# e-c-k-e-r/tortoise-tts

Hardware: AMD Instinct MI355X
Metric: audio-sec/wall-sec (RTF^-1), 16 AR candidates x 80 DDIM steps (higher is better)
Workload: dtype bf16; 1 GPU; configs[1]: 1 utterance/GPU, 64 text tokens, 16 AR candidates x 250 mel tokens (KV-cached decode), latent pass on 16 candidates, 80 DDIM steps with cond-free guidance at T=1088 (11.6 s audio); candidates=16, ddim_steps=80, mel_frames=1088, parallelism=single GPU, small_models=False, vocoder_in_step=False

## Files before the change

### tortoise_tts_amd/csrc/gemm.hip

```cpp
#include <stdlib.h>

#include <type_traits>

#include <hip/hip_ext.h>

#include "gemm_epilogue.h"

namespace ttk {

template <typename T, int BM, int NWM, int NWN, int ROLE>
__device__ __forceinline__ void conv3_image_tile(const GemmParams& p, const int m0, const int n0, const int wave) {
	typedef GRole<ROLE> R;
	static_assert(R::on && R::CONV && R::RES && sizeof(T) == 2, "the k = 3 residual role on 16-bit operands");
	constexpr int ES = 2, BN = 64, KSTEPS = 2, NW = NWM * NWN;
	constexpr int WM = BM / NWM, WN = BN / NWN, MI = WM / 16, NI = WN / 16;
	static_assert(MI == 4 && NI == 2, "64 x 32 wave blocks");
	constexpr int IMG_ROWS = BM + 8, IMG = IMG_ROWS * 128, NPA = IMG_ROWS / 8;
	constexpr int A_PC = (NPA + NW - 1) / NW, B_PC = 8 / NW;
	constexpr int NB = 4, BT = BN * 128, OFF_B = 2 * IMG, OFF_DUMP = OFF_B + NB * BT;
	constexpr int KC = GR_K / 64, NM = KSTEPS * MI * NI, NR = KSTEPS * (MI + NI), RPG = TTK_PIPE_RPG, D0 = TTK_PIPE_D0;
	static_assert(KC % 2 == 0 && (NR + RPG - 1) / RPG <= NM && D0 + B_PC + A_PC <= NM, "reads and DMA pieces must fit the MFMA gaps");
	constexpr unsigned TAPB = (unsigned)(R::N * GR_K * ES);
	constexpr int RESN = MI * 4 * NI;
	constexpr unsigned OOR = 0x80000000u;
	extern __shared__ __attribute__((aligned(16))) char smem[];
	const int lane = threadIdx.x & 63, g = lane >> 4, l15 = lane & 15;
#ifdef TTK_STAMPS
	unsigned long long* const stamps_ = p.stamps;
#endif
	const int wm = wave / NWN, wn = wave % NWN;
	const unsigned smem_base = __builtin_amdgcn_readfirstlane(lds_addr(smem));
	const int Tb = p.rows_per_batch;
	float bias_pre[NI];
#pragma unroll
	for (int j = 0; j < NI; ++j) bias_pre[j] = p.bias[n0 + wn * WN + 16 * j + l15];

	unsigned fa[3][KSTEPS], fb[KSTEPS];
#pragma unroll
	for (int ks = 0; ks < KSTEPS; ++ks) {
#pragma unroll
		for (int sg = 0; sg < 3; ++sg) {
			const int r = wm * WM + l15 + sg;
			fa[sg][ks] = smem_base + r * 128 + (((4 * ks + g) ^ (r & 7)) << 4);
		}
		const int rowb = wn * WN + l15;
		fb[ks] = smem_base + OFF_B + rowb * 128 + (((4 * ks + g) ^ (rowb & 7)) << 4);
	}
	const int prow = lane >> 3, pslot = lane & 7;
	unsigned va[A_PC], vb[B_PC];
#pragma unroll
	for (int i = 0; i < A_PC; ++i) {
		const int q = wave + NW * i, r = 8 * q + prow, gr = m0 - 1 + r;
		const bool ok = q < NPA && r < BM + 2 && gr >= 0 && gr < p.M;
		va[i] = ok ? (unsigned)(gr * (GR_K * ES) + ((pslot ^ (r & 7)) << 4)) : OOR;
	}
#pragma unroll
	for (int i = 0; i < B_PC; ++i) {
		const int row = 8 * (wave + NW * i) + prow;
		vb[i] = (unsigned)((n0 + row) * (GR_K * ES) + ((pslot ^ (row & 7)) << 4));
	}
	const __amdgpu_buffer_rsrc_t srdB = __builtin_amdgcn_make_buffer_rsrc((void*)p.W, 0, 0x7fffffff, 0x00020000);
	const __amdgpu_buffer_rsrc_t srdA = __builtin_amdgcn_make_buffer_rsrc((void*)p.seg[0].A, 0, (unsigned)p.M * (unsigned)(GR_K * ES), 0x00020000);
	int mlo = 0, mhi = 0;
#pragma unroll
	for (int i = 0; i < MI; ++i) {
		const int x = m0 + wm * WM + 16 * i + l15;
		const int t = x - div_recip(x, Tb, p.inv_rpb) * Tb;
		mlo |= (t == 0 ? 1 : 0) << i;
		mhi |= (t == Tb - 1 ? 1 : 0) << i;
	}
	const bool any_lo = __builtin_amdgcn_ballot_w64(mlo != 0) != 0, any_hi = __builtin_amdgcn_ballot_w64(mhi != 0) != 0;

	struct PFrags { u32x4 a[KSTEPS][MI], b[KSTEPS][NI]; };
	f32x4 acc[MI][NI];
#pragma unroll
	for (int i = 0; i < MI; ++i)
#pragma unroll
		for (int j = 0; j < NI; ++j) acc[i][j] = f32x4{0.f, 0.f, 0.f, 0.f};

	auto issue_image = [&](auto i_, auto slot_, unsigned kc) {
		constexpr int i = decltype(i_)::value, slot = decltype(slot_)::value;
		const int q = wave + NW * i;
		pipe_glds16(va[i], srdA, kc * 128u, q < NPA ? smem_base + slot * IMG + q * 1024 : smem_base + OFF_DUMP);
	};
	auto issue_w = [&](auto i_, unsigned soff, unsigned slot_off) {
		constexpr int i = decltype(i_)::value;
		pipe_glds16(vb[i], srdB, soff, smem_base + OFF_B + slot_off + (wave + NW * i) * 1024);
	};
	auto read_one = [&](auto r_, auto slot_, auto s_, PFrags& fr, const unsigned (&rb)[KSTEPS]) {
		constexpr int r = decltype(r_)::value, ks = r / (MI + NI), q = r % (MI + NI), SLOT = decltype(slot_)::value, S = decltype(s_)::value;
		if constexpr (q < MI) pipe_read16<q * 2048 + SLOT * IMG>(fr.a[ks][q], fa[S][ks]);
		else pipe_read16<(q - MI) * 2048>(fr.b[ks][q - MI], rb[ks]);
	};
	auto clear_edges = [&](auto s_, PFrags& fr) {
		constexpr int S = decltype(s_)::value;
		if constexpr (S == 0 || S == 2) {
			if (S == 0 ? any_lo : any_hi) {
				const int m = S == 0 ? mlo : mhi;
#pragma unroll
				for (int i = 0; i < MI; ++i) {
					const bool z = (m >> i) & 1;
// ... 15 lines not shown
		unsigned rb[KSTEPS];
#pragma unroll
		for (int ks = 0; ks < KSTEPS; ++ks) rb[ks] = fb[ks] + rd_slot;
		const unsigned soffW = (unsigned)S_CUR * TAPB + kc_w * 128u;
		if constexpr (RD || PER > 0) { wait_vmcnt<W>(); pipe_barrier(); }
		static_for<0, NM>([&](auto m_) {
			constexpr int m = decltype(m_)::value, ks = m / (MI * NI), i = (m % (MI * NI)) / NI, j = m % NI;
			pipe_mfma<T>(acc[i][j], cur.a[ks][i], cur.b[ks][j]);
			if constexpr (RD) static_for<0, RPG>([&](auto q_) {
				constexpr int r = m * RPG + decltype(q_)::value;
				if constexpr (r < NR) read_one(std::integral_constant<int, r>{}, slot_rd_, s_rd_, nxt, rb);
			});
			if constexpr (PER > 0 && m >= D0 && m - D0 < PER) {
				constexpr int d = m - D0;
				if constexpr (ISW && d < B_PC) issue_w(std::integral_constant<int, d>{}, soffW, wr_slot);
				else issue_image(std::integral_constant<int, d - (ISW ? B_PC : 0)>{}, slot_w_, kc_i);
			}
		});
		if constexpr (RD) { pipe_lgkm0(); clear_edges(s_rd_, nxt); }
		tb = (tb + 1) & 3;
	};
	typedef std::integral_constant<int, 0> I0; typedef std::integral_constant<int, 1> I1; typedef std::integral_constant<int, 2> I2;
	typedef std::true_type Y; typedef std::false_type N;

	PipeScope scope = pipe_begin();
	static_for<0, A_PC>([&](auto i_) { issue_image(i_, I0{}, 0u); });
	static_for<0, 3>([&](auto t_) { static_for<0, B_PC>([&](auto i_) { issue_w(i_, (unsigned)decltype(t_)::value * TAPB, (unsigned)decltype(t_)::value * BT); }); });
	static_for<0, A_PC>([&](auto i_) { issue_image(i_, I1{}, 1u); });
	TTK_WSTAMP(stamps_, blockIdx.x, 1);
	wait_vmcnt<2 * B_PC + A_PC>();
	pipe_barrier();
	TTK_WSTAMP(stamps_, blockIdx.x, 2);
	PFrags f0, f1;
	{
		unsigned rb0[KSTEPS];
#pragma unroll
		for (int ks = 0; ks < KSTEPS; ++ks) rb0[ks] = fb[ks];
		static_for<0, NR>([&](auto r_) { read_one(r_, I0{}, I0{}, f0, rb0); });
	}
	pipe_lgkm0();
	clear_edges(I0{}, f0);
	scope.clk = kclock_start();
	typedef std::integral_constant<int, B_PC + A_PC> W01; typedef std::integral_constant<int, B_PC> W2;
	const int row0 = m0 + wm * WM, col0 = n0 + wn * WN;
	float res_pre[MI][4][NI];
	for (int kc = 0; kc < KC - 2; kc += 2) {
		trip(W01{}, Y{}, I0{}, I1{}, Y{}, I0{}, N{}, I0{}, f0, f1, (unsigned)kc + 1, 0u);
		trip(W01{}, Y{}, I0{}, I2{}, Y{}, I1{}, N{}, I0{}, f1, f0, (unsigned)kc + 1, 0u);
		trip(W2{}, Y{}, I1{}, I0{}, Y{}, I2{}, Y{}, I0{}, f0, f1, (unsigned)kc + 1, (unsigned)kc + 2);
		trip(W01{}, Y{}, I1{}, I1{}, Y{}, I0{}, N{}, I1{}, f1, f0, (unsigned)kc + 2, 0u);
		trip(W01{}, Y{}, I1{}, I2{}, Y{}, I1{}, N{}, I1{}, f0, f1, (unsigned)kc + 2, 0u);
		trip(W2{}, Y{}, I0{}, I0{}, Y{}, I2{}, Y{}, I1{}, f1, f0, (unsigned)kc + 2, (unsigned)kc + 3);
	}
	{
		constexpr unsigned kc = KC - 2;
		trip(W01{}, Y{}, I0{}, I1{}, Y{}, I0{}, N{}, I0{}, f0, f1, kc + 1, 0u);
		trip(W01{}, Y{}, I0{}, I2{}, Y{}, I1{}, N{}, I0{}, f1, f0, kc + 1, 0u);
		trip(W2{}, Y{}, I1{}, I0{}, Y{}, I2{}, N{}, I0{}, f0, f1, kc + 1, 0u);
		if (m0 + BM <= p.M) load_residual_role<ROLE, MI, NI, false>(p, res_pre, row0, col0, lane);
		else load_residual_role<ROLE, MI, NI, true>(p, res_pre, row0, col0, lane);
		asm volatile("" ::: "memory");
		TTK_FENCE();
		trip(std::integral_constant<int, B_PC + RESN>{}, Y{}, I1{}, I1{}, N{}, I0{}, N{}, I1{}, f1, f0, 0u, 0u);
		trip(std::integral_constant<int, RESN>{}, Y{}, I1{}, I2{}, N{}, I1{}, N{}, I1{}, f0, f1, 0u, 0u);
		trip(I0{}, N{}, I0{}, I0{}, N{}, I2{}, N{}, I0{}, f1, f0, 0u, 0u);
	}
	pipe_end(scope, TTK_GEMM_STAMPS(p), lane);
	TTK_WSTAMPD(stamps_, blockIdx.x, 3, acc[0][0][0]);
	if (m0 + BM <= p.M) epilogue_role<T, ROLE, false, MI, NI, true>(p, acc, res_pre, bias_pre, row0, col0, lane);
	else epilogue_role<T, ROLE, true, MI, NI, true>(p, acc, res_pre, bias_pre, row0, col0, lane);
	TTK_WSTAMP(stamps_, blockIdx.x, 4);
#if defined(TTK_STAMPS) && TTK_STAMPS == 2
	asm volatile("s_waitcnt vmcnt(0)" ::: "memory");
	TTK_WSTAMP(stamps_, blockIdx.x, 5);
#endif
}

template <typename T, int BM, int BN, int NWM, int NWN, int NSTAGE, int ROLE, bool LONGK = false>
__device__ __forceinline__ void gemm_tile(const GemmParams& p, const int m0, const int n0, const int wave) {
	typedef GRole<ROLE> R;
	static_assert(!R::on || (sizeof(T) <= 2 && R::N % BN == 0), "roles are 16-bit or fp8, N a multiple of the tile width");
	constexpr int LDS_AVAIL = NSTAGE * ((BM == 64 && NWM == 1 ? 128 : BM) + BN) * 128;
	if constexpr (TTK_CONV_IMAGE && R::on && R::CONV && sizeof(T) == 2 && BN == 64 && NWN == 2 && BM / NWM == 64 && LDS_AVAIL >= 2 * (BM + 8) * 128 + 4 * 8192 + 1024) {
		conv3_image_tile<T, BM, NWM, NWN, ROLE>(p, m0, n0, wave);
		return;
	}
	constexpr int ES = sizeof(T);
	constexpr bool F8 = ES == 1;
	constexpr int BKE = 128 / ES;
	constexpr int KSTEPS = F8 ? 2 : BKE / 32;
	constexpr int FCH = F8 ? 1 : 8 * ES / 16;
	constexpr int EPC = 16 / ES;
	constexpr int NW = NWM * NWN;
	constexpr int WM = BM / NWM, WN = BN / NWN, MI = WM / 16, NI = WN / 16;
	constexpr int A_PC = BM / 8 / NW, B_PC = BN / 8 / NW;
	static_assert(A_PC >= 1 && B_PC >= 1 && A_PC * 8 * NW == BM && B_PC * 8 * NW == BN, "tile does not split into 1-KiB pieces per wave");
	constexpr int PER_TILE = A_PC + B_PC;
	constexpr int STAGE = (BM + BN) * 128;
	typedef typename Frag<T>::type FragT;
	extern __shared__ __attribute__((aligned(16))) char smem[];
	const int tid = threadIdx.x, lane = tid & 63;
#ifdef TTK_STAMPS
	unsigned long long* const stamps_ = p.stamps;
#endif
	const int wm = wave / NWN, wn = wave % NWN;
	const int KT = R::on ? GR_K / BKE : p.K / BKE;
	const int NTILES = R::on ? R::NSEG * KT : p.nseg * KT;

	const int prow = lane >> 3, pslot = lane & 7;
	int a_gm[A_PC], a_t[A_PC];
#pragma unroll
	for (int i = 0; i < A_PC; ++i) {
		a_gm[i] = m0 + 8 * (wave + NW * i) + prow;
		if constexpr (R::on) a_t[i] = R::CONV ? a_gm[i] - div_recip(a_gm[i], p.rows_per_batch, p.inv_rpb) * p.rows_per_batch : 0;
		else a_t[i] = p.rows_per_batch > 0 ? a_gm[i] % p.rows_per_batch : 0;
	}
	const unsigned smem_base = __builtin_amdgcn_readfirstlane(lds_addr(smem));
	constexpr unsigned OOR = 0x80000000u;
	unsigned va[A_PC], vb[B_PC];
#pragma unroll
	for (int i = 0; i < B_PC; ++i) {
		const int row = 8 * (wave + NW * i) + prow;
		const int c = pslot ^ (row & 7);
		if constexpr (R::on) vb[i] = (unsigned)((n0 + row) * (GR_K * ES) + c * 16);
		else vb[i] = (unsigned)(((int64_t)(n0 + row) * p.ldw + c * EPC) * ES);
	}
	const __amdgpu_buffer_rsrc_t srdB = __builtin_amdgcn_make_buffer_rsrc((void*)p.W, 0, 0x7fffffff, 0x00020000);
	__amdgpu_buffer_rsrc_t srdA = srdB;
	unsigned b_seg_off = 0;
	int seg_i = 0, kk_i = 0;
	const bool seg_in = R::on ? R::CONV : (p.seg_inner != 0);
	const int NSEG = R::on ? R::NSEG : p.nseg;
	unsigned va3[R::CONV ? 3 : 1][A_PC];
	if constexpr (R::on && R::CONV) {
#pragma unroll
		for (int sg = 0; sg < 3; ++sg)
#pragma unroll
			for (int i = 0; i < A_PC; ++i) {
				const int row = 8 * (wave + NW * i) + prow;
				const int c = pslot ^ (row & 7);
				const int t = a_t[i] + sg - 1;
				const bool ok = a_gm[i] < p.M && t >= 0 && t < p.rows_per_batch;
				va3[sg][i] = ok ? (unsigned)((a_gm[i] + sg - 1) * (GR_K * ES) + c * 16) : OOR;
			}
		srdA = __builtin_amdgcn_make_buffer_rsrc((void*)p.seg[0].A, 0, (unsigned)p.M * (unsigned)(GR_K * ES), 0x00020000);
	}
	auto set_segment = [&](int sg) {
		if constexpr (R::on && R::CONV) {
			b_seg_off = (unsigned)sg * (unsigned)(R::N * GR_K * ES);
#pragma unroll
			for (int i = 0; i < A_PC; ++i) va[i] = sg == 0 ? va3[0][i] : (sg == 1 ? va3[1][i] : va3[2][i]);
			return;
		}
		if constexpr (R::on) {
			srdA = __builtin_amdgcn_make_buffer_rsrc((void*)p.seg[0].A, 0, (unsigned)p.M * (unsigned)(GR_K * ES), 0x00020000);
			b_seg_off = 0;
#pragma unroll
			for (int i = 0; i < A_PC; ++i) {
				const int row = 8 * (wave + NW * i) + prow;
				const int c = pslot ^ (row & 7);
				va[i] = a_gm[i] < p.M ? (unsigned)(a_gm[i] * (GR_K * ES) + c * 16) : OOR;
			}
			return;
		}
		sg = __builtin_amdgcn_readfirstlane(sg);
		const int64_t lda = p.seg[sg].lda;
		const int shift = p.seg[sg].shift;
// ... 351 lines not shown
			asm volatile("s_waitcnt lgkmcnt(0)" ::: "memory");
	#endif
	#if !(defined(TTK_DIAG_SKIP) && (TTK_DIAG_SKIP & 64))
			__builtin_amdgcn_s_barrier();
	#endif
			asm volatile("" ::: "memory");
	#ifdef TTK_DIAG_SKIP
			if ((TTK_DIAG_SKIP & 4) && kt > 0) { if (kt + NSTAGE < NTILES) issue(kt % NSTAGE); mfma_tile(cur); return; }
			if ((TTK_DIAG_SKIP & 8) && kt > 0) { if (kt + NSTAGE < NTILES) issue(kt % NSTAGE); read_frags(nxt, (kt + 1) % NSTAGE); return; }
	#endif
			if (kt + NSTAGE < NTILES) issue(kt % NSTAGE);
			read_frags(nxt, (kt + 1) % NSTAGE);
			mfma_tile(cur);
		};

	#pragma unroll
		for (int st = 0; st < NSTAGE; ++st)
			if (st < NTILES) issue(st);
		TTK_WSTAMP(stamps_, blockIdx.x, 1);
		wait_tiles(min(NSTAGE, NTILES) - 1);
		__builtin_amdgcn_s_barrier();
		asm volatile("" ::: "memory");
		TTK_WSTAMP(stamps_, blockIdx.x, 2);
		Frags f0, f1;
		read_frags(f0, 0);
		if constexpr (PRE_RES) {
			constexpr int NT = R::NSEG * (GR_K / BKE);
			static_assert(!PRE_RES || (NT % 2 == 0 && NT >= 8), "the peeled tail assumes an even tile count");
			auto tail_step = [&](auto wtag, int stage_next, const Frags& cur, Frags& nxt) {
				wait_vmcnt<decltype(wtag)::value>();
	#if !(defined(TTK_DIAG_SKIP) && (TTK_DIAG_SKIP & 32))
				asm volatile("s_waitcnt lgkmcnt(0)" ::: "memory");
	#endif
				__builtin_amdgcn_s_barrier();
				asm volatile("" ::: "memory");
				read_frags(nxt, stage_next);
				mfma_tile(cur);
			};
			int kt = 0;
			for (; kt < NT - 4; kt += 2) {
				step(kt, f0, f1);
				step(kt + 1, f1, f0);
			}
			step(NT - 4, f0, f1);
			if (m0 + BM <= p.M) load_residual_role<ROLE, MI, NI, false>(p, res_pre, row0, col0, lane);
			else load_residual_role<ROLE, MI, NI, true>(p, res_pre, row0, col0, lane);
			asm volatile("" ::: "memory");
			tail_step(std::integral_constant<int, PER_TILE + RESN>{}, (NT - 2) % NSTAGE, f1, f0);
			tail_step(std::integral_constant<int, RESN>{}, (NT - 1) % NSTAGE, f0, f1);
			mfma_tile(f1);
		} else {
			int kt = 0;
			for (; kt + 2 < NTILES; kt += 2) {
				step(kt, f0, f1);
				step(kt + 1, f1, f0);
			}
			if (kt + 2 == NTILES) { step(kt, f0, f1); mfma_tile(f1); }
			else mfma_tile(f0);
		}
	}
	TTK_WSTAMPD(stamps_, blockIdx.x, 3, acc[0][0][0]);

	if constexpr (R::on) {
		if (m0 + BM <= p.M) epilogue_role<T, ROLE, false, MI, NI, PRE_RES>(p, acc, res_pre, bias_pre, row0, col0, lane);
		else epilogue_role<T, ROLE, true, MI, NI, PRE_RES>(p, acc, res_pre, bias_pre, row0, col0, lane);
		TTK_WSTAMP(stamps_, blockIdx.x, 4);
#if defined(TTK_STAMPS) && TTK_STAMPS == 2
		asm volatile("s_waitcnt vmcnt(0)" ::: "memory");
		TTK_WSTAMP(stamps_, blockIdx.x, 5);
#endif
		return;
	}
	const bool full = (m0 + BM <= p.M) && (n0 + BN <= p.N);
	if (p.transpose_out) { if (full) epilogue<T, 2, false, MI, NI>(p, acc, row0, col0, lane); else epilogue<T, 2, true, MI, NI>(p, acc, row0, col0, lane); }
	else if (p.out_f32) { if (full) epilogue<T, 1, false, MI, NI>(p, acc, row0, col0, lane); else epilogue<T, 1, true, MI, NI>(p, acc, row0, col0, lane); }
	else { if (full) epilogue<T, 0, false, MI, NI>(p, acc, row0, col0, lane); else epilogue<T, 0, true, MI, NI>(p, acc, row0, col0, lane); }
	TTK_WSTAMP(stamps_, blockIdx.x, 4);
#if defined(TTK_STAMPS) && TTK_STAMPS == 2
	asm volatile("s_waitcnt vmcnt(0)" ::: "memory");
	TTK_WSTAMP(stamps_, blockIdx.x, 5);
#endif
}

template <typename B> __device__ __forceinline__ int xcd_tile_id(B block, int nwg) {
	const int xcd = block & 7, q = nwg >> 3, r = nwg & 7;
	return (xcd < r ? xcd * (q + 1) : r * (q + 1) + (xcd - r) * q) + (block >> 3);
}

template <typename T, int BM, int BN, int NWM, int NWN, int NSTAGE, int ROLE = GR_NONE, bool LONGK = false>
__global__ __launch_bounds__(64 * NWM * NWN, 2) void k_gemm(GemmParams p) {
	typedef GRole<ROLE> R;

	if constexpr (R::on) {
		if constexpr (R::CONV) TTK_PIN_ARGS(TTK_S(p.M), TTK_S(p.W), TTK_S(p.seg[0].A), TTK_S(p.tiles_m), TTK_S(p.inv_tiles_m), TTK_S(p.rows_per_batch), TTK_S(p.inv_rpb));
		else TTK_PIN_ARGS(TTK_S(p.M), TTK_S(p.W), TTK_S(p.seg[0].A), TTK_S(p.tiles_m), TTK_S(p.inv_tiles_m));
	} else {
		TTK_PIN_ARGS(TTK_S(p.M), TTK_S(p.N), TTK_S(p.K), TTK_S(p.nseg), TTK_S(p.W), TTK_S(p.ldw), TTK_S(p.rows_per_batch), TTK_S(p.m_major),
					 TTK_S(p.seg[0].A), TTK_S(p.seg[0].lda), TTK_S(p.seg[0].shift), TTK_S(p.seg[0].w_off));
	}
	const int wave = __builtin_amdgcn_readfirstlane((int)threadIdx.x >> 6);
#ifdef TTK_STAMPS
	unsigned long long* const stamps_ = p.stamps;
#endif
	TTK_WSTAMP(stamps_, blockIdx.x, 0);
	const int tiles_m = R::on ? p.tiles_m : (p.M + BM - 1) / BM;
	const int tile_id = xcd_tile_id(blockIdx.x, R::on ? tiles_m * (R::N / BN) : (int)gridDim.x);
	int m0, n0;
	if constexpr (R::on) {
		const int tn = div_recip(tile_id, tiles_m, p.inv_tiles_m);
		m0 = (tile_id - tn * tiles_m) * BM; n0 = tn * BN;
	} else {
		const int tiles_n = (p.N + BN - 1) / BN;
		m0 = p.m_major ? (tile_id / tiles_n) * BM : (tile_id % tiles_m) * BM;
		n0 = p.m_major ? (tile_id % tiles_n) * BN : (tile_id / tiles_m) * BN;
	}
	gemm_tile<T, BM, BN, NWM, NWN, NSTAGE, ROLE, LONGK>(p, m0, n0, wave);
}

template <typename T, int ROLE>
__global__ __launch_bounds__(256, 2) void k_gemm_mixed(GemmParams p) {
	typedef GRole<ROLE> R;
	static_assert(R::on && R::N == 1024, "mixed grids serve the 1024-wide roles");
	if constexpr (R::CONV) TTK_PIN_ARGS(TTK_S(p.M), TTK_S(p.W), TTK_S(p.seg[0].A), TTK_S(p.mix_full), TTK_S(p.mix_fm), TTK_S(p.inv_tiles_m),
										TTK_S(p.rows_per_batch), TTK_S(p.inv_rpb));
	else TTK_PIN_ARGS(TTK_S(p.M), TTK_S(p.W), TTK_S(p.seg[0].A), TTK_S(p.mix_full), TTK_S(p.mix_fm), TTK_S(p.inv_tiles_m));
	const int wave = __builtin_amdgcn_readfirstlane((int)threadIdx.x >> 6);
#ifdef TTK_STAMPS
	unsigned long long* const stamps_ = p.stamps;
#endif
	TTK_WSTAMP(stamps_, blockIdx.x, 0);
	const int b = blockIdx.x;
	if (b < p.mix_full) {
		const int tile_id = xcd_tile_id(b, p.mix_full);
		const int tn = div_recip(tile_id, p.mix_fm, p.inv_tiles_m);
		gemm_tile<T, 128, 64, 2, 2, TTK_ROLE_STAGES, ROLE>(p, (tile_id - tn * p.mix_fm) * 128, tn * 64, wave);
	} else {
		if (wave >= 2) return;
		const int j = b - p.mix_full;
		gemm_tile<T, 64, 64, 1, 2, TTK_ROLE_STAGES, ROLE>(p, p.mix_fm * 128 + (j >> 4) * 64, (2 * (j & 7) + ((j >> 3) & 1)) * 64, wave);
	}
}

static void opt_in_lds_once(bool& done, const void* kernel, int lds) {
	if (done) return;
	if (lds > 64 * 1024) (void)hipFuncSetAttribute(kernel, hipFuncAttributeMaxDynamicSharedMemorySize, lds);
	done = true;
}
static void fill_derived(GemmParams& p, int tiles_m) {
	p.tiles_m = tiles_m;
	p.inv_tiles_m = 1.0f / (float)tiles_m;
	p.inv_rpb = p.rows_per_batch > 0 ? 1.0f / (float)p.rows_per_batch : 0.f;
	p.inv_gn_T = p.gn_T > 0 ? 1.0f / (float)p.gn_T : 0.f;
}

template <typename T, int BM, int BN, int NWM, int NWN, int NSTAGE, int ROLE = GR_NONE, bool LONGK = false>
static void launch_tile(const GemmParams& p_in, hipStream_t s, hipEvent_t ea, hipEvent_t eb) {
	constexpr int LDS = NSTAGE * (BM + BN) * 128;
	if constexpr (!LONGK && ROLE == GR_NONE && sizeof(T) == 2 && BM == 256 && BN == 128 && NSTAGE == 3) {
		if (TTK_GEMM_PIPE_H && (p_in.K / 64) * p_in.nseg > NSTAGE) return launch_tile<T, BM, BN, NWM, NWN, NSTAGE, ROLE, true>(p_in, s, ea, eb);
	}
	static bool attr_set = false;
	opt_in_lds_once(attr_set, (const void*)k_gemm<T, BM, BN, NWM, NWN, NSTAGE, ROLE, LONGK>, LDS);
	GemmParams p = p_in;
	fill_derived(p, (p.M + BM - 1) / BM);
	const int grid = p.tiles_m * ((p.N + BN - 1) / BN);
	hipExtLaunchKernelGGL((k_gemm<T, BM, BN, NWM, NWN, NSTAGE, ROLE, LONGK>), dim3(grid), dim3(64 * NWM * NWN), (unsigned)LDS, s, ea, eb, 0, p);
}

static int g_mixed_mode = -1;
static bool mixed_grid_applies(const GemmParams& p) {
	if (g_mixed_mode < 0) { const char* e = getenv("TTK_GEMM_MIXED"); g_mixed_mode = e ? atoi(e) : 1; }
	if (!g_mixed_mode || p.N != 1024 || p.M % 64 != 0) return false;
	const int tiles_m = (p.M + 127) / 128;
	return tiles_m * 16 > 256 && tiles_m * 16 <= 320;
}
template <typename T, int ROLE>
static void launch_mixed(const GemmParams& p_in, hipStream_t s, hipEvent_t ea, hipEvent_t eb) {
	constexpr int LDS = TTK_ROLE_STAGES * (128 + 64) * 128;
	static_assert(LDS > 64 * 1024, "the mixed grid's ring needs the LDS opt-in");
	static bool attr_set = false;
	opt_in_lds_once(attr_set, (const void*)k_gemm_mixed<T, ROLE>, LDS);
	GemmParams p = p_in;
	p.mix_fm = 16; p.mix_full = 256;
	fill_derived(p, p.mix_fm);
	const int blocks64 = (p.M - 128 * p.mix_fm) / 64;
	hipExtLaunchKernelGGL((k_gemm_mixed<T, ROLE>), dim3(p.mix_full + blocks64 * 16), dim3(256), (unsigned)LDS, s, ea, eb, 0, p);
}

int g_gemm_roles = -1;
void gemm_roles_refresh() {
	g_mixed_mode = -1;
	const char* e = getenv("TTK_GEMM_ROLE");
	g_gemm_roles = e ? (atoi(e) == 1 ? 0x1E : atoi(e)) : 0x1E;
}
static int gemm_role_of_unmasked(const GemmParams& p, int es);
static int gemm_role_of(const GemmParams& p, int es) {
	const int r = gemm_role_of_unmasked(p, es);
	return (g_gemm_roles >> r) & 1 ? r : GR_NONE;
}
static int gemm_role_of_unmasked(const GemmParams& p, int es) {
	if (g_gemm_roles < 0) gemm_roles_refresh();
	if ((es != 2 && es != 1) || p.K != GR_K || p.ldw != GR_K || !p.bias || p.act != ACT_NONE || (es == 2) != (p.out_scale == 0.f)) return GR_NONE;
	if (p.transpose_out || p.m_major) return GR_NONE;
	if (p.M < 1 || p.M > (1 << 19) || p.seg[0].lda != GR_K || p.seg[0].w_off != 0) return GR_NONE;
	if (p.nseg == 1 && p.seg[0].shift == 0) {
		if (p.N == 3072 && !p.out_f32 && p.ldc == 3072 && !p.residual && !p.gn_part) return GR_QKV;
		if (p.N == 1024 && p.out_f32 && p.ldc == 1024 && p.gn_part && p.gn_T > 0) return !p.residual ? GR_IN1x1 : (p.ldr == 1024 ? GR_PROJ_RES : GR_NONE);
		return GR_NONE;
	}
	if (p.nseg == 3 && p.N == 1024 && p.out_f32 && p.ldc == 1024 && p.residual && p.ldr == 1024 && p.gn_part && p.gn_T > 0 && p.rows_per_batch > 0) {
		for (int j = 0; j < 3; ++j)
			if (p.seg[j].A != p.seg[0].A || p.seg[j].lda != GR_K || p.seg[j].shift != j - 1 || p.seg[j].w_off != (int64_t)j * 1024 * GR_K) return GR_NONE;
		return GR_CONV3_RES;
	}
	return GR_NONE;
}
static bool is_stat_role(int role) { return role == GR_IN1x1 || role == GR_CONV3_RES || role == GR_PROJ_RES; }
template <typename F> static void with_stat_role(int role, F&& f) {
	if (role == GR_IN1x1) f(std::integral_constant<int, GR_IN1x1>{});
	else if (role == GR_CONV3_RES) f(std::integral_constant<int, GR_CONV3_RES>{});
	else if (role == GR_PROJ_RES) f(std::integral_constant<int, GR_PROJ_RES>{});
}
template <typename T, int BM, int BN, int NWM, int NWN, int NSTAGE>
static void launch_tile_role(int role, const GemmParams& p, hipStream_t s, hipEvent_t ea, hipEvent_t eb) {
	if constexpr (sizeof(T) <= 2) {
		if constexpr (BM == 128 && BN == 64) {
			if (is_stat_role(role) && mixed_grid_applies(p)) return with_stat_role(role, [&](auto r) { launch_mixed<T, decltype(r)::value>(p, s, ea, eb); });
		}
		constexpr int NS = (BM == 128 && BN == 64 && sizeof(T) == 2) ? TTK_ROLE_STAGES : NSTAGE;
		if constexpr (BN <= 128) {
			if (is_stat_role(role)) return with_stat_role(role, [&](auto r) { launch_tile<T, BM, BN, NWM, NWN, NS, decltype(r)::value>(p, s, ea, eb); });
		}
		if (role == GR_QKV) return launch_tile<T, BM, BN, NWM, NWN, NS, GR_QKV>(p, s, ea, eb);
	}
	launch_tile<T, BM, BN, NWM, NWN, NSTAGE>(p, s, ea, eb);
}

int g_force_tile = -1;
static void read_force_tile() { if (g_force_tile < 0) { const char* e = getenv("TTK_GEMM_TILE"); g_force_tile = e ? atoi(e) + 100 : 99; } }
static int pick_tile(int M, int N) {
	const int t128 = ((M + 127) / 128) * ((N + 127) / 128);
	const int t12864 = ((M + 127) / 128) * ((N + 63) / 64);
	return t128 >= 256 ? 0 : (t12864 >= 128 ? 1 : 2);
}
bool gemm_fuses_gn_stats(int M, int N, int C, int T) {
	read_force_tile();
	if (g_force_tile >= 100 && g_force_tile - 100 == 2) return false;
	return C == 1024 && N == C && T % 64 == 0 && M % 64 == 0 && pick_tile(M, N) != 2;
}

template <typename T>
static void launch_gemm_t(const GemmParams& p, hipStream_t s, hipEvent_t ea, hipEvent_t eb) {
	read_force_tile();
	int tile;
	if (g_force_tile >= 100) tile = g_force_tile - 100;
	else {
		tile = pick_tile(p.M, p.N);
	}
	static const int wide = [] { const char* e = getenv("TTK_GEMM_TILE_WIDE"); return e ? atoi(e) : -2; }();
	if (g_force_tile < 100 && tile == 0) {
		const int t128 = ((p.M + 127) / 128) * ((p.N + 127) / 128), t256 = ((p.M + 255) / 256) * ((p.N + 127) / 128);
		if (wide >= 0) { if (p.N >= 3072) tile = wide; }
		else if (wide == -2 && sizeof(T) <= 2 && t128 > 256) {
			const int r128 = (t128 + 255) / 256, r256 = (t256 + 255) / 256;
			if (15 * r256 <= 9 * r128) tile = 8;
		}
	}
	const int role = gemm_role_of(p, (int)sizeof(T));
	if (tile == 0) launch_tile_role<T, 128, 128, 2, 4, 3>(role, p, s, ea, eb);
	else if (tile == 1) launch_tile_role<T, 128, 64, 2, 2, 3>(role, p, s, ea, eb);
	else if (tile == 3) launch_tile<T, 128, 128, 2, 4, 4>(p, s, ea, eb);
	else if (tile == 4) launch_tile<T, 128, 64, 2, 2, 5>(p, s, ea, eb);
	else if (tile == 5) launch_tile<T, 128, 64, 4, 2, 3>(p, s, ea, eb);
	else if (tile == 6) launch_tile<T, 128, 64, 2, 4, 3>(p, s, ea, eb);
	else if (tile == 7) launch_tile<T, 256, 64, 4, 2, 3>(p, s, ea, eb);
	else if (tile == 8) launch_tile_role<T, 256, 128, 4, 2, 3>(role, p, s, ea, eb);
	else if (tile == 9) launch_tile<T, 128, 128, 2, 4, 2>(p, s, ea, eb);
	else launch_tile<T, 64, 64, 2, 2, 3>(p, s, ea, eb);
}

void launch_gemm(int dt, const GemmParams& p_in, hipStream_t s) {
	static const int order = [] { const char* e = getenv("TTK_GEMM_ORDER"); return e ? atoi(e) : 0; }();
	GemmParams p = p_in;
	if (order == 1) p.m_major = p.nseg == 1 && (int64_t)p.N < p.M;
	else if (order == 2) p.m_major = (int64_t)p.N * p.nseg < p.M;
	else if (order == 3) p.m_major = 1;
	p.seg_inner = p.nseg == 3 && p.seg[0].shift == -1 && p.seg[1].shift == 0 && p.seg[2].shift == 1 && p.seg[1].A == p.seg[0].A && p.seg[2].A == p.seg[0].A &&
				  p.seg[1].lda == p.seg[0].lda && p.seg[2].lda == p.seg[0].lda;
	hipEvent_t ea = nullptr, eb = nullptr;
	if (g_prof_on) prof_pair(PROF_GEMM, 2.0 * p.M * p.N * (double)p.K * p.nseg, &ea, &eb);
	if (dt == DT_FP8) launch_gemm_t<f8>(p, s, ea, eb);
	else if (dt == DT_BF16) launch_gemm_t<bf16>(p, s, ea, eb);
	else if (dt == DT_F16) launch_gemm_t<f16>(p, s, ea, eb);
	else launch_gemm_t<float>(p, s, ea, eb);
}

}
```

### tortoise_tts_amd/csrc/gemm_prims.h

```cpp
#pragma once

#include <type_traits>

#include "ttk_common.h"
#include "ttk_kernels.h"

#ifndef TTK_GEMM_PIPE
#define TTK_GEMM_PIPE 1
#endif
#ifndef TTK_GEMM_PIPE_H
#define TTK_GEMM_PIPE_H 1
#endif
#ifndef TTK_CONV_IMAGE
#define TTK_CONV_IMAGE 1
#endif
#ifndef TTK_ROLE_STAGES
#define TTK_ROLE_STAGES 3
#endif
#ifndef TTK_FP8_SCALED_MFMA
#define TTK_FP8_SCALED_MFMA 1
#endif
#ifndef TTK_PIPE_RPG
#define TTK_PIPE_RPG 2
#endif
#ifndef TTK_PIPE_PREB
#define TTK_PIPE_PREB 0
#endif
#ifndef TTK_PIPE_DPG
#define TTK_PIPE_DPG 1
#endif
#ifndef TTK_PIPE_DLATE
#define TTK_PIPE_DLATE 0
#endif
#ifndef TTK_PIPE_D0
#define TTK_PIPE_D0 6
#endif

#ifdef TTK_STAMPS
#define TTK_GEMM_STAMPS(p) ((p).stamps)
#else
#define TTK_GEMM_STAMPS(p) ((unsigned long long*)nullptr)
#endif

namespace ttk {

__device__ __forceinline__ void glds16(unsigned voff, __amdgpu_buffer_rsrc_t srd, unsigned soff, unsigned lds_dst ) {
	unsigned keep;
	asm volatile("s_mov_b32 %0, m0\n\ts_mov_b32 m0, %1\n\ts_nop 0\n\tbuffer_load_dwordx4 %2, %3, %4 offen lds\n\ts_mov_b32 m0, %0"
				 : "=&s"(keep) : "s"(lds_dst), "v"(voff), "s"(srd), "s"(soff) : "memory");
}
__device__ __forceinline__ unsigned lds_addr(const void* p) {
	return (unsigned)(uintptr_t)(const __attribute__((address_space(3))) char*)p;
}
template <int N> __device__ __forceinline__ void wait_vmcnt() { asm volatile("s_waitcnt vmcnt(%0)" ::"n"(N) : "memory"); }
template <int I, int N, typename F> __device__ __forceinline__ void static_for(F&& f) {
	if constexpr (I < N) { f(std::integral_constant<int, I>{}); static_for<I + 1, N>(f); }
}

typedef __attribute__((ext_vector_type(4))) unsigned u32x4;
#define TTK_FENCE() __builtin_amdgcn_sched_barrier(0)
template <int OFF> __device__ __forceinline__ void pipe_read16(u32x4& d, unsigned addr) {
	static_assert(OFF >= 0 && OFF < 65536, "ds_read offset field");
	asm volatile("ds_read_b128 %0, %1 offset:%2" : "=v"(d) : "v"(addr), "n"(OFF));
	TTK_FENCE();
}
template <typename T> __device__ __forceinline__ void pipe_mfma(f32x4& c, const u32x4& a, const u32x4& b) {
	union U { u32x4 q; typename Frag<T>::type v; __device__ U() {} } ua, ub;
	ua.q = a; ub.q = b;
	c = mma16<T>(ua.v, ub.v, c);
	TTK_FENCE();
}
__device__ __forceinline__ void pipe_lgkm0() { asm volatile("s_waitcnt lgkmcnt(0)" ::: "memory"); TTK_FENCE(); }
__device__ __forceinline__ void pipe_barrier() { TTK_FENCE(); __builtin_amdgcn_s_barrier(); asm volatile("" ::: "memory"); TTK_FENCE(); }
__device__ __forceinline__ void pipe_glds16(unsigned voff, __amdgpu_buffer_rsrc_t srd, unsigned soff, unsigned lds_dst ) {
	asm volatile("s_mov_b32 m0, %0\n\ts_nop 0\n\tbuffer_load_dwordx4 %1, %2, %3 offen lds" :: "s"(lds_dst), "v"(voff), "s"(srd), "s"(soff) : "memory");
	TTK_FENCE();
}
#ifdef TTK_CLOCK_STAMPS
struct KClock { unsigned long long clk0, rt0; };
__device__ __forceinline__ KClock kclock_start() { return KClock{__builtin_amdgcn_s_memtime(), __builtin_amdgcn_s_memrealtime()}; }
__device__ __forceinline__ void kclock_stop(const KClock& c, unsigned long long* stamps, int lane) {
	if (stamps && lane == 0) {
		unsigned long long* st_ = stamps + ((size_t)blockIdx.x * 16 + (threadIdx.x >> 6)) * 8;
		st_[6] = ((__builtin_amdgcn_s_memtime() - c.clk0) << 32) | ((__builtin_amdgcn_s_memrealtime() - c.rt0) & 0xffffffffull);
	}
}
#else
struct KClock {};
__device__ __forceinline__ KClock kclock_start() { return KClock{}; }
__device__ __forceinline__ void kclock_stop(const KClock&, unsigned long long*, int) {}
#endif
__device__ __forceinline__ unsigned pipe_m0_save() { unsigned k; asm volatile("s_mov_b32 %0, m0" : "=s"(k)); TTK_FENCE(); return k; }
__device__ __forceinline__ void pipe_m0_restore(unsigned k) { asm volatile("s_mov_b32 m0, %0" :: "s"(k)); TTK_FENCE(); }
struct PipeScope { unsigned m0_keep; KClock clk; };
__device__ __forceinline__ PipeScope pipe_begin() {
	PipeScope s;
	asm volatile("s_mov_b32 %0, m0" : "=s"(s.m0_keep));
	TTK_FENCE();
	return s;
}
// ... 8 lines not shown
```

### tortoise_tts_amd/csrc/ttk_kernels.h

```cpp
#pragma once
#include <hip/hip_runtime.h>
#include <stdint.h>

namespace ttk {

enum DType { DT_F32 = 0, DT_BF16 = 1, DT_FP8W = 2, DT_FP8 = 3, DT_F16 = 4 };
inline int elem_kind(int dt) { return dt == DT_F32 ? 1 : (dt == DT_F16 ? 2 : 0); }
inline size_t dtype_size(int dt) { return dt == DT_F32 ? 4 : 2; }
inline int kernel_dtype(int dt) { return (dt == DT_FP8W || dt == DT_FP8) ? DT_BF16 : dt; }

enum ProfKind { PROF_GEMM = 0, PROF_SKINNY = 1, PROF_ATTN_FWD = 2, PROF_ATTN_DECODE = 3, PROF_GN_STATS = 4, PROF_GN_APPLY = 5,
				PROF_LAYERNORM = 6, PROF_KINDS = 7 };
extern bool g_prof_on;
void prof_start(int kind, double work, hipStream_t s);
void prof_stop(hipStream_t s);
void prof_pair(int kind, double work, hipEvent_t* start, hipEvent_t* stop);
struct ProfScope {
	hipStream_t s; bool on;
	ProfScope(int kind, double work, hipStream_t s_) : s(s_), on(g_prof_on) { if (on) prof_start(kind, work, s); }
	~ProfScope() { if (on) prof_stop(s); }
};

struct GemmSeg {
	const void* A;
	int64_t lda;
	int shift;
	int64_t w_off;
};
struct GemmParams {
	int nseg;
	int M, N, K;
	const void* W;
	int64_t ldw;
	int rows_per_batch;
	int act;
	const float* bias;
	const float* residual;
	int64_t ldr;
	void* C;
	int64_t ldc;
	float out_scale;
	int out_f32;
	int transpose_out;
	int gn_T; float* gn_part;
	int seg_inner;
	int m_major;
	int tiles_m; float inv_tiles_m, inv_rpb, inv_gn_T;
	int mix_full, mix_fm;
#ifdef TTK_STAMPS
	unsigned long long* stamps;
#endif
	GemmSeg seg[12];
};
enum GemmRole { GR_NONE = 0, GR_IN1x1 = 1, GR_CONV3_RES = 2, GR_QKV = 3, GR_PROJ_RES = 4 };
void launch_gemm(int dt, const GemmParams& p, hipStream_t s);
void gemm_roles_refresh();
bool gemm_fuses_gn_stats(int M, int N, int C, int T);

enum SkinnyMode { SK_STORE_F32 = 0, SK_RESIDUAL = 1, SK_ACT_T = 2, SK_QKV = 3 };
struct SkinnyParams {
	const void* Wp;
	int N, K, M;
	const float* bias;
	int ln_count;
	const float* x;  int64_t ldx;
	const float* g1;
	union {
		const float* b1;
		int* health;
	};
	const float *g2, *b2;
	const void* a;
	int mode, act;
	float* out_f32;  int64_t ldc;
	void* out_T;
	float* qbuf; void* kcache; void* vcache; int max_ctx, H; float q_scale;
	const int* d_pos;
	float* noise; const void* rng; const int64_t* draws;
	int w8; float wscale;
#ifdef TTK_STAMPS
	unsigned long long* stamps;
#endif
};
enum SkinnyForm { SKF_PLAIN = 0, SKF_FOLD = 1, SKF_PROLOGUE = 2 };
constexpr size_t CU_LDS_BYTES = 160 * 1024;
constexpr size_t LDS_DEFAULT_LIMIT = 64 * 1024;
inline int skinny_launch_waves(int waves, bool prologue) { return waves < 4 ? 4 : (prologue && waves > 8 ? 8 : waves); }
inline size_t skinny_lds_bytes(int dt, int MT, int K, int waves, int form) {
	const size_t red = (size_t)waves * MT * 64 * 4 * sizeof(float);
	if (form == SKF_PROLOGUE) return (size_t)16 * MT * ((size_t)K * dtype_size(dt) + 16) + red;
	return form == SKF_FOLD ? red + (size_t)waves * MT * 16 * 2 * sizeof(float) : red;
}
hipError_t launch_skinny(int dt, const SkinnyParams& p, int waves, hipStream_t s);

enum GemvRole { GV_QKV = 0, GV_PROJ = 1, GV_FC = 2, GV_HEAD = 3 };
inline int decode_row_tiles(int M) { return M <= 16 ? 1 : (M <= 32 ? 2 : (M <= 48 ? 3 : 4)); }

struct GemvParams {
	const void* Wp;
	const void* a;
	const float* bias;
	const float* csum;
	float* out_f32;
	void* out_T;
	float* qbuf; void* kcache; void* vcache;
	const int* d_pos;
	float* noise; const void* rng; const int64_t* draws;
	int* health;
	int M, N, max_ctx, H, row0;
	float q_scale, wscale;
	int K, w8;
#ifdef TTK_STAMPS
	unsigned long long* stamps;
#endif
};
bool launch_gemv(int dt, int role, const GemvParams& p, hipStream_t s);
bool gemv_supported(int dt, int role, const GemvParams& p);

void launch_layernorm(int dt, const float* x, int64_t ldx, int rows, int d, const float* g1, const float* b1,
					  const float* g2, const float* b2, void* out, int64_t ldo, int out_f32, hipStream_t s, int frag = 0, float* out2 = nullptr,
					  const int64_t* out2_idx = nullptr, int64_t out2_stride = 0, const int64_t* out2_base = nullptr);
int gn_num_chunks(int T, int C);
int gn_rows_per_chunk(int C);
void launch_gn_stats(const float* x, int nb, int T, int C, float* part, hipStream_t s, const int* tlen = nullptr, const int* need = nullptr);
struct GnApplyParams {
	const float* x; const float* ms; const float* gamma; const float* beta;
	const float* scale; const float* shift; int64_t ss_stride;
	const int* row_idx; int nb, T, Tout, C; int nchunks; int act; void* out; int out_f32;
	const int* tlen; int chunk_rows;
	int out_f8;
	const void* pf; int64_t pf_bytes; int pf_taps;
// ... 82 lines not shown
```

Before: 40.43 audio-sec/wall-sec.

## Add even-grid plan mixing wide and narrow tiles for 1024-wide role GEMMs

Adds a compile-time tile plan for N=1024 role GEMMs with 17-32 row strips. Some blocks compute double-width 128x128 tiles (8 waves) and the rest compute 128x64 tiles, so the total block count fits within 256 CUs in a single wave. The aim is to remove the tail effect and wave quantization of the previous mixed grid. In exchange, block size grows to 512 threads with a larger LDS opt-in. Inactive waves in narrow blocks exit early, which could hurt occupancy or per-tile efficiency.

```diff
diff --git a/tortoise_tts_amd/csrc/gemm.hip b/tortoise_tts_amd/csrc/gemm.hip
--- a/tortoise_tts_amd/csrc/gemm.hip
+++ b/tortoise_tts_amd/csrc/gemm.hip
@@ -8,15 +8,16 @@
 
 namespace ttk {
 
-template <typename T, int BM, int NWM, int NWN, int ROLE>
+template <typename T, int BM, int BN, int NWM, int NWN, int ROLE>
 __device__ __forceinline__ void conv3_image_tile(const GemmParams& p, const int m0, const int n0, const int wave) {
 	typedef GRole<ROLE> R;
 	static_assert(R::on && R::CONV && R::RES && sizeof(T) == 2, "the k = 3 residual role on 16-bit operands");
-	constexpr int ES = 2, BN = 64, KSTEPS = 2, NW = NWM * NWN;
+	constexpr int ES = 2, KSTEPS = 2, NW = NWM * NWN;
 	constexpr int WM = BM / NWM, WN = BN / NWN, MI = WM / 16, NI = WN / 16;
-	static_assert(MI == 4 && NI == 2, "64 x 32 wave blocks");
+	static_assert(MI == 4 && NI == 2 && (BN == 64 || BN == 128), "64 x 32 wave blocks");
 	constexpr int IMG_ROWS = BM + 8, IMG = IMG_ROWS * 128, NPA = IMG_ROWS / 8;
-	constexpr int A_PC = (NPA + NW - 1) / NW, B_PC = 8 / NW;
+	constexpr int A_PC = (NPA + NW - 1) / NW, B_PC = BN / 8 / NW;
+	static_assert(B_PC * 8 * NW == BN, "a weight tile splits into whole pieces per wave");
 	constexpr int NB = 4, BT = BN * 128, OFF_B = 2 * IMG, OFF_DUMP = OFF_B + NB * BT;
 	constexpr int KC = GR_K / 64, NM = KSTEPS * MI * NI, NR = KSTEPS * (MI + NI), RPG = TTK_PIPE_RPG, D0 = TTK_PIPE_D0;
 	static_assert(KC % 2 == 0 && (NR + RPG - 1) / RPG <= NM && D0 + B_PC + A_PC <= NM, "reads and DMA pieces must fit the MFMA gaps");
@@ -198,7 +199,7 @@
 	static_assert(!R::on || (sizeof(T) <= 2 && R::N % BN == 0), "roles are 16-bit or fp8, N a multiple of the tile width");
 	constexpr int LDS_AVAIL = NSTAGE * ((BM == 64 && NWM == 1 ? 128 : BM) + BN) * 128;
 	if constexpr (TTK_CONV_IMAGE && R::on && R::CONV && sizeof(T) == 2 && BN == 64 && NWN == 2 && BM / NWM == 64 && LDS_AVAIL >= 2 * (BM + 8) * 128 + 4 * 8192 + 1024) {
-		conv3_image_tile<T, BM, NWM, NWN, ROLE>(p, m0, n0, wave);
+		conv3_image_tile<T, BM, 64, NWM, NWN, ROLE>(p, m0, n0, wave);
 		return;
 	}
 	constexpr int ES = sizeof(T);
@@ -716,7 +717,7 @@
 #endif
 }
 
-template <typename B> __device__ __forceinline__ int xcd_tile_id(B block, int nwg) {
+template <typename B> __host__ __device__ constexpr int xcd_tile_id(B block, int nwg) {
 	const int xcd = block & 7, q = nwg >> 3, r = nwg & 7;
 	return (xcd < r ? xcd * (q + 1) : r * (q + 1) + (xcd - r) * q) + (block >> 3);
 }
@@ -751,27 +752,92 @@
 	gemm_tile<T, BM, BN, NWM, NWN, NSTAGE, ROLE, LONGK>(p, m0, n0, wave);
 }
 
+constexpr int EVEN_R0 = 17, EVEN_R1 = 32;
+constexpr int even_grid_f(int R) {
+	for (int f = TTK_EVEN_F; f <= 8; ++f)
+		if (R * (16 - f) <= 256) return f;
+	return -1;
+}
+constexpr int even_grid_blocks(int R) { return R * (16 - even_grid_f(R)); }
+constexpr bool even_grid_widened(int R, int f, int strip, int pair) { return ((pair + R * f - strip * f) & 7) < f; }
+constexpr unsigned EVEN_WIDE = 512;
+struct EvenGrid { unsigned e[EVEN_R1 - EVEN_R0 + 1][256]; };
+constexpr EvenGrid make_even_grid() {
+	EvenGrid g{};
+	for (int R = EVEN_R0; R <= EVEN_R1; ++R) {
+		const int f = even_grid_f(R), nw = R * f;
+		unsigned* e = g.e[R - EVEN_R0];
+		for (int b = 0; b < nw; ++b) e[b] = (unsigned)(b / f) | (unsigned)(2 * ((b + 7 * nw) & 7)) << 5 | EVEN_WIDE;
+		unsigned order[256] = {};
+		int nn = 0;
+		for (int c = 0; c < 16; ++c)
+			for (int s = 0; s < R; ++s)
+				if (!even_grid_widened(R, f, s, c >> 1)) order[nn++] = (unsigned)s | (unsigned)c << 5;
+		for (int j = 0; j < nn; ++j) e[nw + j] = order[xcd_tile_id(j, nn)];
+	}
+	return g;
+}
+constexpr EvenGrid kEvenGrid = make_even_grid();
+constexpr bool even_grid_ok(int R) {
+	const int f = even_grid_f(R), blocks = even_grid_blocks(R);
+	if (f < 0 || f > 8 || blocks > 256) return false;
+	int cover[EVEN_R1][16] = {};
+	for (int b = 0; b < blocks; ++b) {
+		const unsigned e = kEvenGrid.e[R - EVEN_R0][b];
+		const int s = e & 31, c = (e >> 5) & 15;
+		if (s >= R) return false;
+		++cover[s][c];
+		if (e & EVEN_WIDE) { if (c & 1) return false; ++cover[s][c + 1]; }
+	}
+	for (int s = 0; s < R; ++s)
+		for (int c = 0; c < 16; ++c)
+			if (cover[s][c] != 1) return false;
+	return true;
+}
+static_assert(even_grid_ok(17) && even_grid_ok(18) && even_grid_ok(19) && even_grid_ok(24) && even_grid_ok(31) && even_grid_ok(32), "the even grid's plan");
+#if TTK_EVEN_F == 0
+static_assert(even_grid_f(17) == 1 && even_grid_blocks(17) == 255 && even_grid_f(19) == 3 && even_grid_blocks(19) == 247 && even_grid_f(24) == 6 &&
+			  even_grid_blocks(24) == 240 && even_grid_f(32) == 8 && even_grid_blocks(32) == 256, "the even grid's plan");
+#endif
+__device__ const EvenGrid g_even_grid = make_even_grid();
+
+template <typename T, int ROLE> constexpr bool even_wide_image() { return TTK_CONV_IMAGE && GRole<ROLE>::CONV && sizeof(T) == 2; }
+template <typename T, int ROLE> constexpr int even_grid_lds() {
+	constexpr int narrow = TTK_ROLE_STAGES * (128 + 64) * 128, wide = even_wide_image<T, ROLE>() ? 2 * (128 + 8) * 128 + 4 * 128 * 128 + 1024 : 3 * (128 + 128) * 128;
+	return narrow > wide ? narrow : wide;
+}
+
 template <typename T, int ROLE>
-__global__ __launch_bounds__(256, 2) void k_gemm_mixed(GemmParams p) {
+__global__ __launch_bounds__(512, 2) void k_gemm_mixed(GemmParams p) {
 	typedef GRole<ROLE> R;
-	static_assert(R::on && R::N == 1024, "mixed grids serve the 1024-wide roles");
-	if constexpr (R::CONV) TTK_PIN_ARGS(TTK_S(p.M), TTK_S(p.W), TTK_S(p.seg[0].A), TTK_S(p.mix_full), TTK_S(p.mix_fm), TTK_S(p.inv_tiles_m),
-										TTK_S(p.rows_per_batch), TTK_S(p.inv_rpb));
-	else TTK_PIN_ARGS(TTK_S(p.M), TTK_S(p.W), TTK_S(p.seg[0].A), TTK_S(p.mix_full), TTK_S(p.mix_fm), TTK_S(p.inv_tiles_m));
+	static_assert(R::on && R::N == 1024, "these grids serve the 1024-wide roles");
+	if constexpr (R::CONV) TTK_PIN_ARGS(TTK_S(p.M), TTK_S(p.W), TTK_S(p.seg[0].A), TTK_S(p.mix_plan), TTK_S(p.rows_per_batch), TTK_S(p.inv_rpb));
+	else TTK_PIN_ARGS(TTK_S(p.M), TTK_S(p.W), TTK_S(p.seg[0].A), TTK_S(p.mix_plan));
 	const int wave = __builtin_amdgcn_readfirstlane((int)threadIdx.x >> 6);
 #ifdef TTK_STAMPS
 	unsigned long long* const stamps_ = p.stamps;
 #endif
 	TTK_WSTAMP(stamps_, blockIdx.x, 0);
 	const int b = blockIdx.x;
-	if (b < p.mix_full) {
-		const int tile_id = xcd_tile_id(b, p.mix_full);
-		const int tn = div_recip(tile_id, p.mix_fm, p.inv_tiles_m);
-		gemm_tile<T, 128, 64, 2, 2, TTK_ROLE_STAGES, ROLE>(p, (tile_id - tn * p.mix_fm) * 128, tn * 64, wave);
+	if (p.mix_plan < 0) {
+		if (b < 256) {
+			const int tile_id = xcd_tile_id(b, 256);
+			gemm_tile<T, 128, 64, 2, 2, TTK_ROLE_STAGES, ROLE>(p, (tile_id & 15) * 128, (tile_id >> 4) * 64, wave);
+		} else {
+			if (wave >= 2) return;
+			const int j = b - 256;
+			gemm_tile<T, 64, 64, 1, 2, TTK_ROLE_STAGES, ROLE>(p, 2048 + (j >> 4) * 64, (2 * (j & 7) + ((j >> 3) & 1)) * 64, wave);
+		}
+		return;
+	}
+	const unsigned e = g_even_grid.e[p.mix_plan][b];
+	const int m0 = (int)(e & 31) * 128, n0 = (int)((e >> 5) & 15) * 64;
+	if (e & EVEN_WIDE) {
+		if constexpr (even_wide_image<T, ROLE>()) conv3_image_tile<T, 128, 128, 2, 4, ROLE>(p, m0, n0, wave);
+		else gemm_tile<T, 128, 128, 2, 4, 3, ROLE>(p, m0, n0, wave);
 	} else {
-		if (wave >= 2) return;
-		const int j = b - p.mix_full;
-		gemm_tile<T, 64, 64, 1, 2, TTK_ROLE_STAGES, ROLE>(p, p.mix_fm * 128 + (j >> 4) * 64, (2 * (j & 7) + ((j >> 3) & 1)) * 64, wave);
+		if (wave >= 4) return;
+		gemm_tile<T, 128, 64, 2, 2, TTK_ROLE_STAGES, ROLE>(p, m0, n0, wave);
 	}
 }
 
@@ -802,23 +868,29 @@
 }
 
 static int g_mixed_mode = -1;
-static bool mixed_grid_applies(const GemmParams& p) {
+static int mixed_grid_mode(const GemmParams& p) {
 	if (g_mixed_mode < 0) { const char* e = getenv("TTK_GEMM_MIXED"); g_mixed_mode = e ? atoi(e) : 1; }
-	if (!g_mixed_mode || p.N != 1024 || p.M % 64 != 0) return false;
-	const int tiles_m = (p.M + 127) / 128;
-	return tiles_m * 16 > 256 && tiles_m * 16 <= 320;
+	if (!g_mixed_mode || p.N != 1024 || p.M % 64 != 0) return 0;
+	const int strips = (p.M + 127) / 128;
+	if (strips < EVEN_R0 || strips >= EVEN_R1) return 0;
+	return strips <= 20 && g_mixed_mode != 2 ? 1 : 2;
 }
 template <typename T, int ROLE>
-static void launch_mixed(const GemmParams& p_in, hipStream_t s, hipEvent_t ea, hipEvent_t eb) {
-	constexpr int LDS = TTK_ROLE_STAGES * (128 + 64) * 128;
-	static_assert(LDS > 64 * 1024, "the mixed grid's ring needs the LDS opt-in");
+static void launch_mixed(int mode, const GemmParams& p_in, hipStream_t s, hipEvent_t ea, hipEvent_t eb) {
+	constexpr int LDS_HALF = TTK_ROLE_STAGES * (128 + 64) * 128, LDS_EVEN = even_grid_lds<T, ROLE>();
+	static_assert(LDS_HALF > 64 * 1024 && LDS_EVEN > 80 * 1024 && LDS_EVEN <= 160 * 1024, "the rings need the LDS opt-in; one workgroup of the even grid per CU");
 	static bool attr_set = false;
-	opt_in_lds_once(attr_set, (const void*)k_gemm_mixed<T, ROLE>, LDS);
+	opt_in_lds_once(attr_set, (const void*)k_gemm_mixed<T, ROLE>, LDS_EVEN);
 	GemmParams p = p_in;
-	p.mix_fm = 16; p.mix_full = 256;
-	fill_derived(p, p.mix_fm);
-	const int blocks64 = (p.M - 128 * p.mix_fm) / 64;
-	hipExtLaunchKernelGGL((k_gemm_mixed<T, ROLE>), dim3(p.mix_full + blocks64 * 16), dim3(256), (unsigned)LDS, s, ea, eb, 0, p);
+	const int strips = (p.M + 127) / 128;
+	fill_derived(p, strips);
+	if (mode == 1) {
+		p.mix_plan = -1;
+		hipExtLaunchKernelGGL((k_gemm_mixed<T, ROLE>), dim3(256 + (p.M - 2048) / 64 * 16), dim3(256), (unsigned)LDS_HALF, s, ea, eb, 0, p);
+	} else {
+		p.mix_plan = strips - EVEN_R0;
+		hipExtLaunchKernelGGL((k_gemm_mixed<T, ROLE>), dim3(even_grid_blocks(strips)), dim3(512), (unsigned)LDS_EVEN, s, ea, eb, 0, p);
+	}
 }
 
 int g_gemm_roles = -1;
@@ -859,7 +931,8 @@
 static void launch_tile_role(int role, const GemmParams& p, hipStream_t s, hipEvent_t ea, hipEvent_t eb) {
 	if constexpr (sizeof(T) <= 2) {
 		if constexpr (BM == 128 && BN == 64) {
-			if (is_stat_role(role) && mixed_grid_applies(p)) return with_stat_role(role, [&](auto r) { launch_mixed<T, decltype(r)::value>(p, s, ea, eb); });
+			const int mode = is_stat_role(role) ? mixed_grid_mode(p) : 0;
+			if (mode) return with_stat_role(role, [&](auto r) { launch_mixed<T, decltype(r)::value>(mode, p, s, ea, eb); });
 		}
 		constexpr int NS = (BM == 128 && BN == 64 && sizeof(T) == 2) ? TTK_ROLE_STAGES : NSTAGE;
 		if constexpr (BN <= 128) {
diff --git a/tortoise_tts_amd/csrc/gemm_prims.h b/tortoise_tts_amd/csrc/gemm_prims.h
--- a/tortoise_tts_amd/csrc/gemm_prims.h
+++ b/tortoise_tts_amd/csrc/gemm_prims.h
@@ -16,6 +16,9 @@
 #endif
 #ifndef TTK_ROLE_STAGES
 #define TTK_ROLE_STAGES 3
+#endif
+#ifndef TTK_EVEN_F
+#define TTK_EVEN_F 0
 #endif
 #ifndef TTK_FP8_SCALED_MFMA
 #define TTK_FP8_SCALED_MFMA 1
diff --git a/tortoise_tts_amd/csrc/ttk_kernels.h b/tortoise_tts_amd/csrc/ttk_kernels.h
--- a/tortoise_tts_amd/csrc/ttk_kernels.h
+++ b/tortoise_tts_amd/csrc/ttk_kernels.h
@@ -46,7 +46,7 @@
 	int seg_inner;
 	int m_major;
 	int tiles_m; float inv_tiles_m, inv_rpb, inv_gn_T;
-	int mix_full, mix_fm;
+	int mix_plan;
 #ifdef TTK_STAMPS
 	unsigned long long* stamps;
 #endif
```

Result: no change. 40.37 audio-sec/wall-sec, median of 2 (-0.1%).
